# yhwu/rsicnv

Measured on AMD Instinct MI355X. Metric: bases/sec through RSI pipeline (bin+GC+NB+segment), higher is better.
Workload: dtype int32

## Files before the change

rsicnv_amd/csrc/kernels.h:

```cpp
#pragma once
#include <hip/hip_runtime.h>
#include <stdint.h>
#include <mutex>
#include "device_util.h"

namespace rsik {

inline void note_launch() {
  const hipError_t e = hipGetLastError();
  if (e != hipSuccess && tl_launch_error == hipSuccess) tl_launch_error = e;
}
inline void drain_stale_errors() { (void)hipGetLastError(); tl_launch_error = hipSuccess; }
inline hipError_t take_launch_error() { const hipError_t e = tl_launch_error; tl_launch_error = hipSuccess; return e; }
#define RSI_LAUNCH(...) do { hipLaunchKernelGGL(__VA_ARGS__); rsik::note_launch(); } while (0)

constexpr int kGcLevels = 202;
constexpr int kHistValues = 65536;
constexpr int kResClasses = 32;
constexpr int kTileBases = 4096;

void launch_fasta_classify(const uint8_t* fasta, int64_t n, uint64_t* gcbits, uint64_t* nbits, int64_t nwords,
                           const FillList& fill, hipStream_t stream);
void launch_fill(const FillList& fill, hipStream_t stream);
size_t fold_scratch_bytes();
// ... 185 lines not shown
#define RSI_ALLOW_FULL_LDS(kernel)                                                                                  \
  do {                                                                                                              \
    static std::once_flag once__[rsik::kMaxDevices];                                                                \
    int dev__ = 0;                                                                                                  \
    if (hipGetDevice(&dev__) != hipSuccess || dev__ < 0 || dev__ >= rsik::kMaxDevices) dev__ = 0;                   \
    std::call_once(once__[dev__], [dev__] {                                                                         \
      hipFuncAttributes a__;                                                                                        \
      int lds__ = 0;                                                                                                \
      if (hipFuncGetAttributes(&a__, reinterpret_cast<const void*>(kernel)) != hipSuccess) {                        \
        rsik::report_attribute_failure(#kernel, "hipFuncGetAttributes"); return;                                    \
      }                                                                                                             \
      if (hipDeviceGetAttribute(&lds__, hipDeviceAttributeMaxSharedMemoryPerBlock, dev__) != hipSuccess || lds__ <= 0) \
        lds__ = 160 * 1024;                                                                                         \
      if (hipFuncSetAttribute(reinterpret_cast<const void*>(kernel), hipFuncAttributeMaxDynamicSharedMemorySize,   \
                              lds__ - (int)a__.sharedSizeBytes) != hipSuccess)                                      \
        rsik::report_attribute_failure(#kernel, "hipFuncSetAttribute(MaxDynamicSharedMemorySize)");                 \
    });                                                                                                             \
  } while (0)

constexpr unsigned kCandHistBins = 16384;
struct EdgeJob {
  int32_t start, end, type, pad;
};
struct CandJob {
  int32_t start, end;
  int32_t kind;
  int32_t margin;
  int32_t capacity;
  int32_t top;
  int32_t nleft, nright;
  int32_t left_off, right_off;
  int32_t budget;
  int32_t cut;
  double right_cap;
  int64_t iscratch_off;
  int64_t lscratch_off;
};
struct CandOut {
  int32_t flags;
  int32_t nref, nbody, nwin, left_reach, right_reach, body_min, body_max;
  double body_q[3], body_s1, body_s2;
  double ref_q[3], ref_s1, ref_s2;
};
struct DepthRef { const void* p; int bytes; };
void launch_widen_u8(const uint8_t* src, int64_t n, int32_t* dst, hipStream_t stream);
void launch_patch_i32(int32_t* dst, const int32_t* pos, const int32_t* val, int64_t cnt, hipStream_t stream);
void launch_range_sums(DepthRef rdc, const void* ranges , int nranges, long long* sums, hipStream_t stream);
void launch_sharpen_edges(DepthRef rdc, int64_t ncompact, EdgeJob* jobs, int njobs, void* ws, int ws_jobs, hipStream_t stream);
size_t sharpen_workspace_bytes(int njobs);
size_t sharpen_workspace_zero_bytes(int njobs);
constexpr int kCandChunks = 16;
struct CandMid {
  int32_t lcnt, lreach, lused, rcnt_max, rreach, rused;
  uint32_t done, body_flags;
  long long totals[kCandChunks];
  float flo[kCandChunks], fhi[kCandChunks];
  double m1[kCandChunks], m2[kCandChunks];
  int32_t body_min, body_max;
  double body_q[3], body_s1, body_s2;
};
void launch_candidate_test_split(DepthRef rdc, int64_t ncompact, const CandJob* jobs, int njobs, const void* chains,
                                 int32_t* iscratch, long long* lscratch, double RDmedian, CandMid* mid, uint32_t* ghist,
                                 CandOut* outs, hipStream_t stream);
void launch_candidate_test(DepthRef rdc, int64_t ncompact, const CandJob* jobs, int njobs, const void* chains,
                           int32_t* iscratch, long long* lscratch, double RDmedian, CandOut* outs, hipStream_t stream);

struct TextParseStats { unsigned long long lines, stored, beyond; unsigned int unsorted, pad; };
int text_parse_workgroups(long long nbytes);
void launch_parse_depth_text(const void* text, long long nbytes, long long size, int32_t* depth, long long* wg_first,
                             long long* wg_max, TextParseStats* stats, hipStream_t stream);

struct NameBound { long long line; int32_t name, len; };
void launch_text_name_bounds(const void* text, long long nbytes, NameBound* bounds, unsigned int* count, unsigned int cap,
                             hipStream_t stream, bool bedgraph = false);
struct GenomeSeg { long long start, n; int32_t* depth; int32_t slot, pad; };
struct GenomeSlotStats { unsigned long long lines, stored, beyond; unsigned int unsorted, pad; long long last_pos;  };
constexpr int kMaxGenomeSegs = 512;
int genome_parse_workgroups(long long nbytes);
void launch_parse_genome_text(const void* text, long long begin, long long end, const GenomeSeg* segs, int nseg,
                              GenomeSlotStats* slots, long long* wg, hipStream_t stream);
constexpr int kMaxGenomeSamples = 64;
struct GenomeSampleCols { int32_t col[kMaxGenomeSamples], j[kMaxGenomeSamples]; int32_t n, pad; };
__host__ __device__ inline long long genome_sample_stride(long long n) { return (n + 4 + 3) & ~3ll; }
int genome_sample_parse_workgroups(long long nbytes);
void launch_parse_genome_samples(const void* text, long long begin, long long end, const GenomeSeg* segs, int nseg,
                                 const GenomeSampleCols& cols, GenomeSlotStats* slots, long long* wg, hipStream_t stream);
struct BedRun { int32_t* dst; uint32_t len; int32_t d; };
constexpr long long kBedPiece = 1ll << 20;
unsigned long long bedgraph_run_cap(long long text_bytes, long long sum_len);
void launch_parse_genome_bedgraph(const void* text, long long begin, long long end, const GenomeSeg* segs, int nseg, GenomeSlotStats* slots,
                                  long long* wg, BedRun* runs, unsigned long long* nruns, unsigned int run_cap, hipStream_t stream);

struct InflateBlock { long long coff, out; uint32_t clen, isize, crc, pad; };
void launch_inflate_bgzf(const void* comp, const InflateBlock* blocks, int nblocks, void* text, int* last_nl,
                         unsigned long long* status, hipStream_t stream);
void launch_gather_names(const void* text, const NameBound* bounds, unsigned k0, unsigned k1, char* out, hipStream_t stream);
// ... 9 lines not shown
```

rsicnv_amd/csrc/kernels_cand.hip:

```cpp
#include "kernels.h"

namespace rsik {

namespace {

constexpr int kThreads = 256;
constexpr int kTestThreads = 1024;
constexpr int kMaxWaves = kTestThreads / 64;
__device__ inline int lane_id() { return threadIdx.x & 63; }

template <class T, class Op>
__device__ inline T block_reduce(T v, Op op, T* s_tmp ) {
  for (int d = 32; d >= 1; d >>= 1) v = op(v, __shfl_xor(v, d));
  __syncthreads();
  if (lane_id() == 0) s_tmp[threadIdx.x >> 6] = v;
  __syncthreads();
  T r = s_tmp[0];
  for (int w = 1; w < (int)(blockDim.x >> 6); ++w) r = op(r, s_tmp[w]);
  __syncthreads();
  return r;
}
__device__ inline int block_exscan(int v, int* s_tmp , int* total) {
  const int incl = wave_incl_scan(v);
  __syncthreads();
  if (lane_id() == 63) s_tmp[threadIdx.x >> 6] = incl;
  __syncthreads();
  int base = 0, tot = 0;
  for (int w = 0; w < (int)(blockDim.x >> 6); ++w) { if (w < (int)(threadIdx.x >> 6)) base += s_tmp[w]; tot += s_tmp[w]; }
  __syncthreads();
  *total = tot;
  return base + incl - v;
}
template <class F>
// ... 143 lines not shown

constexpr int kWalkPer = 16;
constexpr int kWalkBlock = kWalkPer * kTestThreads;

struct WalkShared { int s_scan[kMaxWaves]; int cnt[2][kMaxWaves]; int trg[2][kMaxWaves]; int kept[2]; int lastt[2]; };

struct __attribute__((packed, aligned(1))) WalkBytes16 { uint32_t w[4]; };
struct __attribute__((packed, aligned(4))) WalkInts4 { int x, y, z, w; };
__device__ inline void walk_load16(const uint8_t* __restrict__ A, int64_t N, long long first, int dir, int* out) {
  const long long lo = dir > 0 ? first : first - 15;
  if (lo >= 0 && lo + 15 <= N - 1) {
    const WalkBytes16 b = *reinterpret_cast<const WalkBytes16*>(A + lo);
#pragma unroll
    for (int j = 0; j < 16; ++j) { const int k = dir > 0 ? j : 15 - j; out[j] = (int)((b.w[k >> 2] >> (8 * (k & 3))) & 0xffu); }
  } else {
#pragma unroll
    for (int j = 0; j < 16; ++j) { long long p = first + (long long)dir * j; p = p < 0 ? 0 : (p > N - 1 ? N - 1 : p); out[j] = (int)A[p]; }
  }
}
__device__ inline void walk_load16(const int32_t* __restrict__ A, int64_t N, long long first, int dir, int* out) {
  const long long lo = dir > 0 ? first : first - 15;
  if (lo >= 0 && lo + 15 <= N - 1) {
    int v[16];
#pragma unroll
    for (int q = 0; q < 4; ++q) { const WalkInts4 b = *reinterpret_cast<const WalkInts4*>(A + lo + 4 * q); v[4 * q] = b.x; v[4 * q + 1] = b.y; v[4 * q + 2] = b.z; v[4 * q + 3] = b.w; }
#pragma unroll
    for (int j = 0; j < 16; ++j) out[j] = v[dir > 0 ? j : 15 - j];
  } else {
#pragma unroll
    for (int j = 0; j < 16; ++j) { long long p = first + (long long)dir * j; p = p < 0 ? 0 : (p > N - 1 ? N - 1 : p); out[j] = A[p]; }
  }
}

template <typename TD>
__device__ inline int gather_side(const TD* __restrict__ A, int64_t N, int dir, int pos, int room ,
                                  int32_t* __restrict__ dst, int first_slot, const int2* __restrict__ chain, int nchain,
                                  int kind, double too_high, double too_low, WalkShared& W, int* reach, int* chain_used,
                                  int* __restrict__ stage ) {
  constexpr int kNone = 0x7fffffff;
  auto swz = [](int r) { return r ^ ((r >> 4) & 15); };
  int stored = 0, ci = 0, trip = 0;
  int last = pos;
  const int lane = lane_id(), wave = threadIdx.x >> 6, nwaves = blockDim.x >> 6;
  const double th = too_high > 2147483646.0 ? 2147483646.0 : (too_high < -2147483647.0 ? -2147483647.0 : floor(too_high));
  const double tl = too_low > 2147483646.0 ? 2147483646.0 : (too_low < -2147483647.0 ? -2147483647.0 : ceil(too_low));
  const int hi_lim = kind == 0 && too_high == too_high ? (too_high > 2147483646.0 ? 0x7fffffff : (int)th) : 0x7fffffff;
  const int lo_lim = kind == 1 && too_low == too_low ? (too_low < -2147483647.0 ? (int)0x80000000 : (int)tl) : (int)0x80000000;
  auto load16 = [&](int from, int* out) { walk_load16(A, N, (long long)from + (long long)dir * (1 + kWalkPer * (int)threadIdx.x), dir, out); };
  int vnext[kWalkPer];
  load16(pos, vnext);
  int2 cur = ci < nchain ? chain[ci] : make_int2(1, 0);
  while (room > 0 && (dir < 0 ? pos > 2 : (int64_t)pos < N - 2)) {
    const int par = trip & 1;
    ++trip;
    const int avail = dir < 0 ? pos - 2 : (int)(N - 2 - pos);
    const int cnt = avail < kWalkBlock ? avail : kWalkBlock;
    int v[kWalkPer]; unsigned accm = 0; int nacc = 0; int trig = kNone;
#pragma unroll
    for (int j = 0; j < kWalkPer; ++j) v[j] = vnext[j];
    load16(pos + dir * cnt, vnext);
    const int t0 = kWalkPer * (int)threadIdx.x;
#pragma unroll
    for (int j = 0; j < kWalkPer; ++j) {
      const int t = t0 + j;
      if (t < cnt) {
        const int p = pos + dir * (1 + t);
        const bool ext = v[j] > hi_lim || v[j] < lo_lim;
        const bool inside = p >= cur.x && p <= cur.y;
        if (!ext && inside && t < trig) trig = t;
        if (!ext && !inside) { accm |= 1u << j; ++nacc; }
      }
    }
    int incl = wave_incl_scan(nacc), wtrig = trig;
    for (int d = 32; d >= 1; d >>= 1) { const int o = __shfl_xor(wtrig, d); wtrig = o < wtrig ? o : wtrig; }
    if (lane == 63) W.cnt[par][wave] = incl;
    if (lane == 0) W.trg[par][wave] = wtrig;
    __syncthreads();
    int base = 0, all = 0, tstar = kNone;
    for (int w = 0; w < nwaves; ++w) { const int c = W.cnt[par][w]; if (w < wave) base += c; all += c; const int g = W.trg[par][w]; tstar = g < tstar ? g : tstar; }
    int rank = base + incl - nacc;
    int total = all;
    if (tstar != kNone) {
      if ((int)threadIdx.x == tstar / kWalkPer) {
        int k = rank;
#pragma unroll
        for (int j = 0; j < kWalkPer; ++j) if (((accm >> j) & 1u) && t0 + j < tstar) ++k;
        W.kept[par] = k;
      }
      __syncthreads();
// ... 294 lines not shown
  if (room < 0) room = 0;
  g.rcnt = M.rcnt_max < room ? M.rcnt_max : room;
  g.nref_raw = g.used0 + g.rcnt;
  g.nbody = J.end - J.start + 1;
  g.nref = g.nref_raw; g.nbody_eff = g.nbody; g.thin = false;
  if (g.nref_raw + g.nbody > J.budget) {
    const int total = g.nref_raw + g.nbody;
    g.nref = (int)((double)g.nref_raw / (double)total * (double)J.budget);
    g.nbody_eff = (int)((double)g.nbody / (double)total * (double)J.budget);
    g.thin = true;
  }
  g.width = g.nbody_eff;
  g.nwin = g.nref - g.width;
  return g;
}
struct CandBufs { int32_t *left, *ref, *thin, *right; long long* P; };
__device__ inline CandBufs cand_buffers(const CandJob& J, int32_t* iscratch, long long* lscratch) {
  CandBufs b;
  b.left = iscratch + J.iscratch_off;
  b.ref = b.left + (((J.top + 1 > 0 ? J.top + 1 : 0) + 3) & ~3);
  b.thin = b.ref + ((J.capacity + 3) & ~3);
  const int nthin = J.capacity < J.budget ? J.capacity : J.budget;
  b.right = b.thin + ((nthin + 3) & ~3);
  b.P = lscratch + J.lscratch_off;
  return b;
}
__device__ inline int cand_value(const CandJob& J, const CandGeom& g, const CandBufs& b, int i) {
  const int j = g.thin ? (int)((double)i / (double)g.nref * (double)g.nref_raw) : i;
  return j < g.used0 ? b.left[J.top + 1 - g.used0 + j] : b.right[j - g.used0];
}
__device__ inline int cand_chunk_len(int n) { return (((n + kCandChunks - 1) / kCandChunks) + 3) & ~3; }
constexpr int kCandP32MaxChunk = 16000000;

template <typename TD>
__global__ __launch_bounds__(kTestThreads) void k_cand_gather(const TD* __restrict__ A, int64_t N, const CandJob* __restrict__ jobs,
                                                          const int2* __restrict__ chains, int32_t* __restrict__ iscratch,
                                                          long long* __restrict__ lscratch, double RDmedian, CandMid* __restrict__ mid) {
  __shared__ WalkShared W;
  extern __shared__ int s_stage[];
  const CandJob J = jobs[blockIdx.y];
  const CandBufs b = cand_buffers(J, iscratch, lscratch);
  const double too_high = RDmedian * 3.0, too_low = RDmedian * 0.15;
  CandMid& M = mid[blockIdx.y];
  if (blockIdx.x == 0) {
    int lreach = J.start, lused = 0, lcnt = 0;
    if (J.top >= 0)
      lcnt = gather_side(A, N, -1, J.start - J.margin, J.top + 1, b.left, J.top, chains + J.left_off, J.nleft, J.kind, too_high, too_low, W, &lreach, &lused, s_stage);
    if (threadIdx.x == 0) { M.lcnt = lcnt; M.lreach = lreach; M.lused = lused; }
  } else {
    int room = J.capacity;
    const int lim = (int)ceil(J.right_cap);
    if (lim < room) room = lim;
    if ((J.cut & 4) && J.top >= 0) room -= J.top + 1;
    if (room < 0) room = 0;
    int rreach = J.end, rused = 0;
    const int rcnt = gather_side(A, N, +1, J.end + J.margin, room, b.right, 0, chains + J.right_off, J.nright, J.kind, too_high, too_low, W, &rreach, &rused, s_stage);
    if (threadIdx.x == 0) { M.rcnt_max = rcnt; M.rreach = rreach; M.rused = rused; }
  }
}

template <typename TD>
__global__ __launch_bounds__(kTestThreads) void k_cand_prefix(const TD* __restrict__ A, const CandJob* __restrict__ jobs,
                                                          int32_t* __restrict__ iscratch, long long* __restrict__ lscratch,
                                                          CandMid* __restrict__ mid) {
  extern __shared__ unsigned int s_hist[];
  __shared__ long long s_l[kMaxWaves];
  __shared__ int s_i2[kMaxWaves];
  __shared__ int s_scan[kMaxWaves];
  __shared__ int s_q[3];
  const CandJob J = jobs[blockIdx.y];
  CandMid& M = mid[blockIdx.y];
  const CandGeom g = cand_geometry(J, M);
  const CandBufs b = cand_buffers(J, iscratch, lscratch);
  if (g.nwin <= 0 || g.width <= 0) return;
  if (blockIdx.x < kCandChunks) {
    const int Lc = cand_chunk_len(g.nref);
    const int cb = blockIdx.x * Lc;
    int ce = cb + Lc; if (ce > g.nref) ce = g.nref;
    long long carry = 0;
    uint32_t* const P32 = reinterpret_cast<uint32_t*>(b.P);
    const bool p32 = sizeof(TD) == 1 && Lc <= kCandP32MaxChunk;
    if (blockIdx.x == 0 && threadIdx.x == 0) { if (p32) P32[0] = 0u; else b.P[0] = 0; }
    constexpr int kPer = 16;
    for (int t0 = cb; t0 < ce; t0 += kPer * kTestThreads) {
      const int e = t0 + kPer * (int)threadIdx.x;
      int v[kPer];
      if (!g.thin && e + kPer <= ce && (e + kPer <= g.used0 || e >= g.used0)) {
        const int32_t* src = e < g.used0 ? b.left + (J.top + 1 - g.used0 + e) : b.right + (e - g.used0);
#pragma unroll
        for (int q = 0; q < 4; ++q) { const WalkInts4 w4 = *reinterpret_cast<const WalkInts4*>(src + 4 * q); v[4 * q] = w4.x; v[4 * q + 1] = w4.y; v[4 * q + 2] = w4.z; v[4 * q + 3] = w4.w; }
      } else {
// ... 125 lines not shown
  const int Wc = cand_chunk_len(g.nwin);
  const int wb = blockIdx.x * Wc;
  int we = wb + Wc; if (we > g.nwin) we = g.nwin;
  float* Wm = reinterpret_cast<float*>(b.ref);
  const double dw = (double)g.width;
  float flo = 3.0e38f, fhi = -3.0e38f; double m1 = 0, m2 = 0;
  for (int q = wb + (int)threadIdx.x; q < we; q += kTestThreads) {
    const float w = (float)((double)(P_at(q + g.width) - P_at(q)) / dw);
    Wm[q] = w;
    flo = w < flo ? w : flo; fhi = w > fhi ? w : fhi; m1 += (double)w; m2 += (double)w * (double)w;
  }
  flo = block_reduce(flo, [](float a, float b2) { return a < b2 ? a : b2; }, s_f);
  fhi = block_reduce(fhi, [](float a, float b2) { return a > b2 ? a : b2; }, s_f);
  m1 = block_reduce(m1, [](double a, double b2) { return a + b2; }, s_d);
  m2 = block_reduce(m2, [](double a, double b2) { return a + b2; }, s_d);
  if (threadIdx.x == 0) { M.flo[blockIdx.x] = flo; M.fhi[blockIdx.x] = fhi; M.m1[blockIdx.x] = m1; M.m2[blockIdx.x] = m2; }
}

__global__ __launch_bounds__(kTestThreads) void k_cand_hist(const CandJob* __restrict__ jobs, int32_t* __restrict__ iscratch,
                                                        long long* __restrict__ lscratch, CandMid* __restrict__ mid,
                                                        uint32_t* __restrict__ ghist_all, CandOut* __restrict__ outs) {
  extern __shared__ unsigned int s_hist[];
  __shared__ int s_scan[kMaxWaves];
  __shared__ int s_q[3];
  __shared__ int s_last;
  const CandJob J = jobs[blockIdx.y];
  CandMid& M = mid[blockIdx.y];
  const CandGeom g = cand_geometry(J, M);
  const CandBufs b = cand_buffers(J, iscratch, lscratch);
  uint32_t* ghist = ghist_all + (size_t)blockIdx.y * kCandHistBins;
  CandOut O;
  O.flags = M.body_flags;
  if (((J.cut & 1) && M.lused >= J.nleft) || ((J.cut & 2) && M.rused >= J.nright)) O.flags |= 8;
  if ((J.cut & 4) && J.top >= 0 && M.lcnt < J.top + 1) O.flags |= 16;
  O.nref = g.nref; O.nbody = g.nbody_eff; O.nwin = g.nwin; O.left_reach = M.lreach; O.right_reach = M.rreach;
  if (g.nwin <= 0 || g.width <= 0) {
    O.flags = (O.flags & 24) | 1;
    O.body_min = O.body_max = 0; O.body_s1 = O.body_s2 = O.ref_s1 = O.ref_s2 = 0;
    for (int k = 0; k < 3; ++k) { O.body_q[k] = 0; O.ref_q[k] = 0; }
    if (blockIdx.x == 0 && threadIdx.x == 0) outs[blockIdx.y] = O;
    return;
  }
  O.body_min = M.body_min; O.body_max = M.body_max; O.body_s1 = M.body_s1; O.body_s2 = M.body_s2;
  O.body_q[0] = M.body_q[0]; O.body_q[1] = M.body_q[1]; O.body_q[2] = M.body_q[2];
  float flo = 3.0e38f, fhi = -3.0e38f; double m1 = 0, m2 = 0;
  for (int c = 0; c < kCandChunks; ++c) {
    flo = M.flo[c] < flo ? M.flo[c] : flo; fhi = M.fhi[c] > fhi ? M.fhi[c] : fhi; m1 += M.m1[c]; m2 += M.m2[c];
  }
  const double lo = flo, hi = fhi;
  O.ref_s1 = m1; O.ref_s2 = m2;
  O.ref_q[0] = lo; O.ref_q[1] = m1 / (double)g.nwin; O.ref_q[2] = hi;
  const bool spread = (hi - lo) >= 0.01;
  const size_t nbk = spread ? (size_t)((hi - lo) / 0.01 + 2) : 0;
  if (!spread || nbk > kCandHistBins) {
    if (spread) O.flags |= 4;
    if (blockIdx.x == 0 && threadIdx.x == 0) outs[blockIdx.y] = O;
    return;
  }
  const float* Wm = reinterpret_cast<const float*>(b.ref);
  for (unsigned e = threadIdx.x; e < nbk; e += kTestThreads) s_hist[e] = 0;
  __syncthreads();
  const int Wc = cand_chunk_len(g.nwin);
  const int wb = blockIdx.x * Wc;
  int we = wb + Wc; if (we > g.nwin) we = g.nwin;
  for (int i0 = wb + 8 * (int)threadIdx.x; i0 < we; i0 += 8 * kTestThreads) {
    unsigned pend_b = 0xffffffffu, pend_c = 0;
#pragma unroll
// ... 25 lines not shown
}

template <typename TD>
__global__ __launch_bounds__(kThreads) void k_range_sums(const TD* __restrict__ A, const int2* __restrict__ ranges,
                                                         long long* __restrict__ sums) {
  __shared__ long long s_l[kThreads / 64 + 1];
  const int2 r = ranges[blockIdx.x];
  long long acc = 0;
  for (int p = r.x + (int)threadIdx.x; p <= r.y; p += kThreads) acc += A[p];
  acc = block_reduce(acc, [](long long a, long long b) { return a + b; }, s_l);
  if (threadIdx.x == 0) sums[blockIdx.x] = acc;
}

}

#define RSI_DEPTH_DISPATCH(D, CALL32, CALL8) do { if ((D).bytes == 1) { const uint8_t* rdc = static_cast<const uint8_t*>((D).p); CALL8; } \
                                                 else { const int32_t* rdc = static_cast<const int32_t*>((D).p); CALL32; } } while (0)

void launch_range_sums(DepthRef d, const void* ranges, int nranges, long long* sums, hipStream_t stream) {
  if (nranges <= 0) return;
  RSI_DEPTH_DISPATCH(d,
    RSI_LAUNCH(k_range_sums<int32_t>, dim3(nranges), dim3(kThreads), 0, stream, rdc, static_cast<const int2*>(ranges), sums),
    RSI_LAUNCH(k_range_sums<uint8_t>, dim3(nranges), dim3(kThreads), 0, stream, rdc, static_cast<const int2*>(ranges), sums));
}

void launch_sharpen_edges(DepthRef d, int64_t ncompact, EdgeJob* jobs, int njobs, void* ws, int ws_jobs, hipStream_t stream) {
  if (njobs <= 0) return;
  RSI_DEPTH_DISPATCH(d,
    RSI_LAUNCH(k_sharpen_edges<int32_t>, dim3(2 * kEdgeChunks, njobs), dim3(kThreads), 0, stream, rdc, ncompact, jobs, ws_jobs, ws),
    RSI_LAUNCH(k_sharpen_edges<uint8_t>, dim3(2 * kEdgeChunks, njobs), dim3(kThreads), 0, stream, rdc, ncompact, jobs, ws_jobs, ws));
}
void launch_candidate_test_split(DepthRef d, int64_t ncompact, const CandJob* jobs, int njobs, const void* chains,
                                 int32_t* iscratch, long long* lscratch, double RDmedian, CandMid* mid, uint32_t* ghist,
                                 CandOut* outs, hipStream_t stream) {
  if (njobs <= 0) return;
  const size_t lds = (size_t)kCandHistBins * 4;
  static_assert(kCandHistBins * 4 >= (unsigned)kWalkBlock * 4, "the walks stage a trip in the histogram's LDS");
  RSI_ALLOW_FULL_LDS(k_cand_gather<int32_t>);
  RSI_ALLOW_FULL_LDS(k_cand_gather<uint8_t>);
  RSI_ALLOW_FULL_LDS(k_cand_prefix<int32_t>);
  RSI_ALLOW_FULL_LDS(k_cand_prefix<uint8_t>);
  RSI_ALLOW_FULL_LDS(k_cand_hist);
  const int2* ch = static_cast<const int2*>(chains);
  RSI_DEPTH_DISPATCH(d,
    RSI_LAUNCH(k_cand_gather<int32_t>, dim3(2, njobs), dim3(kTestThreads), lds, stream, rdc, ncompact, jobs, ch, iscratch, lscratch, RDmedian, mid),
    RSI_LAUNCH(k_cand_gather<uint8_t>, dim3(2, njobs), dim3(kTestThreads), lds, stream, rdc, ncompact, jobs, ch, iscratch, lscratch, RDmedian, mid));
  RSI_DEPTH_DISPATCH(d,
    RSI_LAUNCH(k_cand_prefix<int32_t>, dim3(kCandChunks + 1, njobs), dim3(kTestThreads), lds, stream, rdc, jobs, iscratch, lscratch, mid),
    RSI_LAUNCH(k_cand_prefix<uint8_t>, dim3(kCandChunks + 1, njobs), dim3(kTestThreads), lds, stream, rdc, jobs, iscratch, lscratch, mid));
  RSI_LAUNCH(k_cand_means, dim3(kCandChunks, njobs), dim3(kTestThreads), 0, stream, jobs, iscratch, lscratch, mid, d.bytes == 1 ? 1 : 0);
  RSI_LAUNCH(k_cand_hist, dim3(kCandChunks, njobs), dim3(kTestThreads), lds, stream, jobs, iscratch, lscratch, mid, ghist, outs);
}
size_t sharpen_workspace_bytes(int njobs) { return sharpen_zero_bytes(njobs) + (size_t)njobs * 2 * kEdgeChunks * (8 + 8 + 4); }
size_t sharpen_workspace_zero_bytes(int njobs) { return sharpen_zero_bytes(njobs); }
void launch_candidate_test(DepthRef d, int64_t ncompact, const CandJob* jobs, int njobs, const void* chains,
                           int32_t* iscratch, long long* lscratch, double RDmedian, CandOut* outs, hipStream_t stream) {
  if (njobs <= 0) return;
  const size_t lds = (size_t)kCandHistBins * 4;
  RSI_ALLOW_FULL_LDS(k_candidate_test<int32_t>);
  RSI_ALLOW_FULL_LDS(k_candidate_test<uint8_t>);
  RSI_DEPTH_DISPATCH(d,
    RSI_LAUNCH(k_candidate_test<int32_t>, dim3(njobs), dim3(kTestThreads), lds, stream, rdc, ncompact, jobs, static_cast<const int2*>(chains), iscratch, lscratch, RDmedian, outs),
    RSI_LAUNCH(k_candidate_test<uint8_t>, dim3(njobs), dim3(kTestThreads), lds, stream, rdc, ncompact, jobs, static_cast<const int2*>(chains), iscratch, lscratch, RDmedian, outs));
}
#undef RSI_DEPTH_DISPATCH

__global__ __launch_bounds__(256) void k_widen_u8(const uint8_t* __restrict__ src, int64_t n, int32_t* __restrict__ dst) {
  const int64_t i0 = ((int64_t)blockIdx.x * 256 + threadIdx.x) * 16;
  if (i0 + 16 <= n) {
    const uint4 b = *reinterpret_cast<const uint4*>(src + i0);
    const uint32_t w[4] = {b.x, b.y, b.z, b.w};
#pragma unroll
    for (int q = 0; q < 4; ++q)
      *reinterpret_cast<int4*>(dst + i0 + 4 * q) = make_int4((int)(w[q] & 0xffu), (int)((w[q] >> 8) & 0xffu), (int)((w[q] >> 16) & 0xffu), (int)(w[q] >> 24));
  } else {
    for (int64_t i = i0; i < n; ++i) dst[i] = (int)src[i];
  }
}
void launch_widen_u8(const uint8_t* src, int64_t n, int32_t* dst, hipStream_t stream) {
  if (n <= 0) return;
  const int64_t blocks = (n + 256 * 16 - 1) / (256 * 16);
  RSI_LAUNCH(k_widen_u8, dim3((unsigned int)blocks), dim3(256), 0, stream, src, n, dst);
}

__global__ __launch_bounds__(256) void k_patch_i32(int32_t* __restrict__ dst, const int32_t* __restrict__ pos, const int32_t* __restrict__ val, int64_t cnt) {
  for (int64_t k = (int64_t)blockIdx.x * 256 + threadIdx.x; k < cnt; k += (int64_t)gridDim.x * 256) dst[pos[k]] = val[k];
}
void launch_patch_i32(int32_t* dst, const int32_t* pos, const int32_t* val, int64_t cnt, hipStream_t stream) {
  if (cnt <= 0) return;
  const int64_t blocks = std::min<int64_t>((cnt + 255) / 256, 1024);
  RSI_LAUNCH(k_patch_i32, dim3((unsigned int)blocks), dim3(256), 0, stream, dst, pos, val, cnt);
// ... 4 lines not shown
```

rsicnv_amd/csrc/pipeline.hip:

```cpp
#include <new>
#include "pipeline_internal.h"

using namespace rsik;
using namespace rsip;
using rsih::Candidate;
using rsih::Region;

namespace {

struct ScanPassOut { uint32_t escapes, inexact, ldel, ldup; };

struct ScanOut {
  double tmedian1 = 0, tsigma1 = 0, tlamda1 = 0, tmedian2 = 0, tsigma2 = 0, tlamda2 = 0;
  int Lmax = 0;
  rsih::IntSpan status2;
  std::vector<int> run_status;
  std::vector<rsih::IntSpan::Range> run_ranges;
  std::vector<Candidate> segs;
  uint32_t escapes = 0, inexact = 0;
  uint32_t tiles_listed = 0;
  std::vector<uint32_t> level_log[4];
  uint32_t stop_levels[4] = {0, 0, 0, 0};
  std::vector<std::string> fs_lines;
};
// ... 201 lines not shown
        if (!ok(ctx->sharpen_ws.ensure(sharpen_workspace_bytes(cap)))) return false;
        if (!ok(hipMemsetAsync(ctx->sharpen_ws.p, 0, sharpen_workspace_zero_bytes(cap), ctx->stream))) return false;
        ctx->sharpen_ws_jobs = cap;
      }
      if (!slot && !ok(ctx->cand_jobs.ensure((size_t)nj * sizeof(EdgeJob)))) return false;
    }
    GateShared gs(ctx);
    Phase ph(ctx, "cand.sharpen");
    EdgeJob* d_jobs = slot ? slot : ctx->cand_jobs.as<EdgeJob>();
    if (!slot && !ok(copy_h2d(ctx, ctx->cand_jobs.p, jobs, (size_t)nj * sizeof(EdgeJob)))) return false;
    for (int pass = 0; pass < 2; ++pass) {
      Timer t(ctx, "sharpen_edges");
      launch_sharpen_edges(d_rdc, N, d_jobs, nj, ctx->sharpen_ws.p, ctx->sharpen_ws_jobs, ctx->stream);
    }
    if (!slot && !ok(copy_d2h(ctx, jobs, ctx->cand_jobs.p, (size_t)nj * sizeof(EdgeJob)))) return false;
    if (!wait()) return false;
    gs.release();
    for (int i = 0; i < nj; ++i) { L[(size_t)i].start = jobs[i].start; L[(size_t)i].end = jobs[i].end; }
    return true;
  }

  bool test(const std::vector<rsih::TestPlan>& plans, std::vector<rsih::TestStats>& stats, std::vector<int>& left_reach,
            std::vector<char>& okv) override {
    const size_t n = plans.size();
    stats.assign(n, rsih::TestStats{});
    left_reach.assign(n, 0);
    okv.assign(n, 0);
    const bool split = env_int("RSI_HOT_CAND_SPLIT", 1) != 0;
    size_t first = 0;
    while (first < n) {
      std::vector<CandJob> jobs;
      std::vector<int32_t> chains;
      size_t iwords = 0, lwords = 0, last = first;
      for (; last < n; ++last) {
        const rsih::TestPlan& T = plans[last];
        if (T.capacity <= 0 || T.end < T.start || T.start < 0 || T.end >= N) break;
        auto up4 = [](size_t x) { return (x + 3) & ~(size_t)3; };
        const size_t iw = up4((size_t)std::max(T.top + 1, 0)) + up4((size_t)T.capacity) + up4((size_t)std::min(T.capacity, T.budget)) +
                          (split ? up4((size_t)T.capacity) : 0);
        const size_t lw = up4((size_t)T.capacity + 1);
        if (!jobs.empty() && (iwords + iw) * 4 + (lwords + lw) * 8 > kCandScratchBytes) break;
        CandJob J{};
        J.start = T.start; J.end = T.end; J.kind = T.kind; J.margin = T.margin; J.capacity = T.capacity; J.top = T.top;
        J.nleft = (int)T.left_chain.size(); J.nright = (int)T.right_chain.size();
        J.left_off = (int)(chains.size() / 2);
        for (const auto& iv : T.left_chain) { chains.push_back(iv.first); chains.push_back(iv.second); }
        J.right_off = (int)(chains.size() / 2);
        for (const auto& iv : T.right_chain) { chains.push_back(iv.first); chains.push_back(iv.second); }
        J.budget = T.budget; J.cut = T.cut; J.right_cap = T.right_cap;
        J.iscratch_off = (int64_t)iwords; J.lscratch_off = (int64_t)lwords;
        iwords += iw; lwords += lw;
        jobs.push_back(J);
      }
      if (jobs.empty()) { ++first; continue; }
      chains.push_back(0); chains.push_back(0);
      std::vector<CandOut> outs(jobs.size());
      {
        Phase ph(ctx, "cand.ensure");
        if (!ok(ctx->cand_jobs.ensure(jobs.size() * sizeof(CandJob))) || !ok(ctx->cand_chains.ensure(chains.size() * 4)) ||
            !ok(ctx->cand_outs.ensure(outs.size() * sizeof(CandOut))) || !ok(ctx->cand_i32.ensure(iwords * 4)) ||
            !ok(ctx->cand_i64.ensure(lwords * 8)))
          return false;
        if (split) {
          const size_t m0 = ctx->cand_mid.cap, h0 = ctx->cand_hist.cap;
          if (!ok(ctx->cand_mid.ensure(jobs.size() * sizeof(CandMid))) || !ok(ctx->cand_hist.ensure(jobs.size() * (size_t)kCandHistBins * 4))) return false;
          if (ctx->cand_mid.cap != m0 && !ok(hipMemsetAsync(ctx->cand_mid.p, 0, ctx->cand_mid.cap, ctx->stream))) return false;
          if (ctx->cand_hist.cap != h0 && !ok(hipMemsetAsync(ctx->cand_hist.p, 0, ctx->cand_hist.cap, ctx->stream))) return false;
        }
      }
      GateShared gs(ctx);
      Phase ph(ctx, "cand.test");
      const size_t jb = (jobs.size() * sizeof(CandJob) + 63) & ~size_t(63), cb = (chains.size() * 4 + 63) & ~size_t(63);
      const size_t ob = outs.size() * sizeof(CandOut);
      unsigned char* slot = jb + cb + ob <= kMailboxMaxCopy ? static_cast<unsigned char*>(mb_alloc(ctx, jb + cb + ob)) : nullptr;
      const CandJob* d_jobs = ctx->cand_jobs.as<CandJob>();
      const void* d_chains = ctx->cand_chains.p;
      CandOut* d_outs = ctx->cand_outs.as<CandOut>();
      if (slot) {
        memcpy(slot, jobs.data(), jobs.size() * sizeof(CandJob));
        memcpy(slot + jb, chains.data(), chains.size() * 4);
        d_jobs = reinterpret_cast<const CandJob*>(slot); d_chains = slot + jb; d_outs = reinterpret_cast<CandOut*>(slot + jb + cb);
      } else {
        if (!ok(copy_h2d(ctx, ctx->cand_jobs.p, jobs.data(), jobs.size() * sizeof(CandJob)))) return false;
        if (!ok(copy_h2d(ctx, ctx->cand_chains.p, chains.data(), chains.size() * 4))) return false;
      }
      {
        Timer t(ctx, split ? "candidate_test" : "candidate_test_one_wg");
        if (split)
          launch_candidate_test_split(d_rdc, N, d_jobs, (int)jobs.size(), d_chains, ctx->cand_i32.as<int32_t>(),
                                      ctx->cand_i64.as<long long>(), median, ctx->cand_mid.as<CandMid>(), ctx->cand_hist.as<uint32_t>(),
                                      d_outs, ctx->stream);
        else
          launch_candidate_test(d_rdc, N, d_jobs, (int)jobs.size(), d_chains, ctx->cand_i32.as<int32_t>(),
                                ctx->cand_i64.as<long long>(), median, d_outs, ctx->stream);
      }
      if (!slot && !ok(copy_d2h(ctx, outs.data(), ctx->cand_outs.p, outs.size() * sizeof(CandOut)))) return false;
      if (!wait()) return false;
      if (slot) memcpy(outs.data(), d_outs, ob);
      gs.release();
      ph.stop();
      static const bool cand_dbg = env_int("RSI_HOT_CAND_DBG", 0) != 0;
      for (size_t k = 0; k < jobs.size(); ++k) {
        const CandOut& O = outs[k];
        if (cand_dbg)
          fprintf(stderr, "[cand] [%d,%d] kind %d margin %d cap %d top %d chains %d/%d cut %d -> flags %d nref %d nbody %d nwin %d reach %d/%d ref q %.6f %.6f %.6f s1 %.6f s2 %.6f\n",
                  jobs[k].start, jobs[k].end, jobs[k].kind, jobs[k].margin, jobs[k].capacity, jobs[k].top, jobs[k].nleft, jobs[k].nright, jobs[k].cut,
                  O.flags, O.nref, O.nbody, O.nwin, O.left_reach, O.right_reach, O.ref_q[0], O.ref_q[1], O.ref_q[2], O.ref_s1, O.ref_s2);
        if (O.flags != 0) continue;
        rsih::TestStats& S = stats[first + k];
        const double nb = (double)O.nbody, nw = (double)O.nwin;
        S.cnv_lqt = O.body_q[0]; S.cnv_med = O.body_q[1]; S.cnv_uqt = O.body_q[2];
        { const double mu = O.body_s1 / nb; S.cnv_var = O.body_s2 / nb - mu * mu; }
        S.ref_lqt = O.ref_q[0]; S.ref_med = O.ref_q[1]; S.ref_uqt = O.ref_q[2];
        { const double mu = O.ref_s1 / nw; S.ref_var = O.ref_s2 / nw - mu * mu; }
        left_reach[first + k] = O.left_reach;
        okv[first + k] = 1;
      }
      first += jobs.size();
    }
    return true;
  }

  bool range_sums(const std::vector<std::pair<int, int>>& ranges, std::vector<int64_t>& sums) override {
    sums.assign(ranges.size(), 0);
    if (ranges.empty()) return true;
    std::vector<int32_t> flat;
    for (const auto& r : ranges) {
      if (r.first < 0 || r.second >= N || r.second < r.first) return false;
      flat.push_back(r.first); flat.push_back(r.second);
    }
    static_assert(sizeof(long long) == sizeof(int64_t), "int64");
    const size_t fb = (flat.size() * 4 + 63) & ~size_t(63);
    unsigned char* slot = static_cast<unsigned char*>(mb_alloc(ctx, fb + ranges.size() * 8));
    GateShared gs(ctx);
    if (slot) {
      memcpy(slot, flat.data(), flat.size() * 4);
      long long* d_sums = reinterpret_cast<long long*>(slot + fb);
      { Timer t(ctx, "range_sums"); launch_range_sums(d_rdc, slot, (int)ranges.size(), d_sums, ctx->stream); }
      if (!wait()) return false;
      memcpy(sums.data(), d_sums, ranges.size() * 8);
// ... 1422 lines not shown
```

Measured before the change: 214.9 billion.

## Parallelize candidate gather walk across tiles with count/scan/scatter kernels

Replaces the two-block-per-job sequential gather walk with a tiled count kernel that counts kept samples per 4096-base tile across many blocks. A last-arriving block scans the tile counts to find where room is filled, resolves chain triggers, and falls back to the old sequential walk when chains overflow or overlap. A separate scatter kernel then writes each tile's kept values at its scanned offset. The host precomputes per-job tile counts to size the grid. The aim is to expose far more parallelism for long walks, at the cost of an extra launch, atomics and more complex fallback logic; one overflow flag is also dropped.

Measured after the change: 208.8 billion (median of 2 runs). -2.8%, worse.

```diff
diff --git a/rsicnv_amd/csrc/kernels.h b/rsicnv_amd/csrc/kernels.h
--- a/rsicnv_amd/csrc/kernels.h
+++ b/rsicnv_amd/csrc/kernels.h
@@ -241,6 +241,7 @@
   int32_t left_off, right_off;
   int32_t budget;
   int32_t cut;
+  int32_t tiles[2];
   double right_cap;
   int64_t iscratch_off;
   int64_t lscratch_off;
@@ -259,9 +260,16 @@
 size_t sharpen_workspace_bytes(int njobs);
 size_t sharpen_workspace_zero_bytes(int njobs);
 constexpr int kCandChunks = 16;
+constexpr int kCandChainMax = 48;
+constexpr int kCandGatherTile = 4096;
 struct CandMid {
   int32_t lcnt, lreach, lused, rcnt_max, rreach, rused;
   uint32_t done, body_flags;
+  uint32_t gdone;
+  int32_t gmode[2];
+  int32_t gstop[2], groom[2];
+  uint32_t walked;
+  uint32_t trig[2][kCandChainMax];
   long long totals[kCandChunks];
   float flo[kCandChunks], fhi[kCandChunks];
   double m1[kCandChunks], m2[kCandChunks];
@@ -270,7 +278,8 @@
 };
 void launch_candidate_test_split(DepthRef rdc, int64_t ncompact, const CandJob* jobs, int njobs, const void* chains,
                                  int32_t* iscratch, long long* lscratch, double RDmedian, CandMid* mid, uint32_t* ghist,
-                                 CandOut* outs, hipStream_t stream);
+                                 CandOut* outs, int max_tiles, hipStream_t stream);
+int cand_gather_tiles(const CandJob& J, const int2* chains, int64_t ncompact, int side);
 void launch_candidate_test(DepthRef rdc, int64_t ncompact, const CandJob* jobs, int njobs, const void* chains,
                            int32_t* iscratch, long long* lscratch, double RDmedian, CandOut* outs, hipStream_t stream);
 
diff --git a/rsicnv_amd/csrc/kernels_cand.hip b/rsicnv_amd/csrc/kernels_cand.hip
--- a/rsicnv_amd/csrc/kernels_cand.hip
+++ b/rsicnv_amd/csrc/kernels_cand.hip
@@ -1,4 +1,7 @@
 #include "kernels.h"
+
+#include <algorithm>
+#include <cmath>
 
 namespace rsik {
 
@@ -208,6 +211,13 @@
   }
 }
 
+__device__ inline void extreme_limits(int kind, double too_high, double too_low, int* hi_lim, int* lo_lim) {
+  const double th = too_high > 2147483646.0 ? 2147483646.0 : (too_high < -2147483647.0 ? -2147483647.0 : floor(too_high));
+  const double tl = too_low > 2147483646.0 ? 2147483646.0 : (too_low < -2147483647.0 ? -2147483647.0 : ceil(too_low));
+  *hi_lim = kind == 0 && too_high == too_high ? (too_high > 2147483646.0 ? 0x7fffffff : (int)th) : 0x7fffffff;
+  *lo_lim = kind == 1 && too_low == too_low ? (too_low < -2147483647.0 ? (int)0x80000000 : (int)tl) : (int)0x80000000;
+}
+
 template <typename TD>
 __device__ inline int gather_side(const TD* __restrict__ A, int64_t N, int dir, int pos, int room ,
                                   int32_t* __restrict__ dst, int first_slot, const int2* __restrict__ chain, int nchain,
@@ -218,10 +228,8 @@
   int stored = 0, ci = 0, trip = 0;
   int last = pos;
   const int lane = lane_id(), wave = threadIdx.x >> 6, nwaves = blockDim.x >> 6;
-  const double th = too_high > 2147483646.0 ? 2147483646.0 : (too_high < -2147483647.0 ? -2147483647.0 : floor(too_high));
-  const double tl = too_low > 2147483646.0 ? 2147483646.0 : (too_low < -2147483647.0 ? -2147483647.0 : ceil(too_low));
-  const int hi_lim = kind == 0 && too_high == too_high ? (too_high > 2147483646.0 ? 0x7fffffff : (int)th) : 0x7fffffff;
-  const int lo_lim = kind == 1 && too_low == too_low ? (too_low < -2147483647.0 ? (int)0x80000000 : (int)tl) : (int)0x80000000;
+  int hi_lim, lo_lim;
+  extreme_limits(kind, too_high, too_low, &hi_lim, &lo_lim);
   auto load16 = [&](int from, int* out) { walk_load16(A, N, (long long)from + (long long)dir * (1 + kWalkPer * (int)threadIdx.x), dir, out); };
   int vnext[kWalkPer];
   load16(pos, vnext);
@@ -230,7 +238,8 @@
     const int par = trip & 1;
     ++trip;
     const int avail = dir < 0 ? pos - 2 : (int)(N - 2 - pos);
-    const int cnt = avail < kWalkBlock ? avail : kWalkBlock;
+    const int trip_len = kWalkPer * (int)blockDim.x;
+    const int cnt = avail < trip_len ? avail : trip_len;
     int v[kWalkPer]; unsigned accm = 0; int nacc = 0; int trig = kNone;
 #pragma unroll
     for (int j = 0; j < kWalkPer; ++j) v[j] = vnext[j];
@@ -591,31 +600,246 @@
 __device__ inline int cand_chunk_len(int n) { return (((n + kCandChunks - 1) / kCandChunks) + 3) & ~3; }
 constexpr int kCandP32MaxChunk = 16000000;
 
+constexpr int kGatherThreads = kCandGatherTile / kWalkPer;
+static_assert(kCandChainMax <= kGatherThreads, "one thread per chain entry");
+struct GatherTileShared {
+  int4 ent[kCandChainMax];
+  int trig[kCandChainMax];
+  int nent;
+  int scan[kMaxWaves];
+  int misc[4];
+};
+struct GatherWalk { int dir, pos0, avail, nchain; const int2* chain; };
+__device__ inline GatherWalk gather_walk(const CandJob& J, int side, int64_t N, const int2* chains) {
+  GatherWalk g;
+  g.dir = side == 0 ? -1 : 1;
+  g.pos0 = side == 0 ? J.start - J.margin : J.end + J.margin;
+  g.avail = side == 0 ? g.pos0 - 2 : (int)(N - 2 - g.pos0);
+  g.chain = chains + (side == 0 ? J.left_off : J.right_off);
+  g.nchain = side == 0 ? J.nleft : J.nright;
+  return g;
+}
+__device__ inline int2 entry_walk(const GatherWalk& g, int2 e) {
+  return g.dir < 0 ? make_int2(g.pos0 - 1 - e.y, g.pos0 - 1 - e.x) : make_int2(e.x - g.pos0 - 1, e.y - g.pos0 - 1);
+}
+__device__ inline int walk_pos(const GatherWalk& g, int t) { return g.pos0 + g.dir * (1 + t); }
+__device__ inline void tile_entries(const GatherWalk& g, int T0, int T1, GatherTileShared& s) {
+  if (threadIdx.x == 0) s.nent = 0;
+  __syncthreads();
+  const int nch = g.nchain < kCandChainMax ? g.nchain : kCandChainMax;
+  if ((int)threadIdx.x < nch) {
+    const int2 w = entry_walk(g, g.chain[threadIdx.x]);
+    if (w.x < T1 && w.y + 1 >= T0) {
+      const int k = atomicAdd(&s.nent, 1);
+      s.ent[k] = make_int4(w.x, w.y, (int)threadIdx.x, 0);
+      s.trig[k] = 0x7fffffff;
+    }
+  }
+  __syncthreads();
+}
+template <typename TD, bool kTrig>
+__device__ inline unsigned tile_taken(const TD* __restrict__ A, int64_t N, const GatherWalk& g, int t0, int T1, int hi_lim, int lo_lim,
+                                      GatherTileShared& s, int* v) {
+  walk_load16(A, N, (long long)walk_pos(g, t0), g.dir, v);
+  unsigned ext = 0;
+#pragma unroll
+  for (int j = 0; j < kWalkPer; ++j) if (t0 + j >= T1 || v[j] > hi_lim || v[j] < lo_lim) ext |= 1u << j;
+  unsigned m = ~ext & 0xffffu;
+  for (int k = 0; k < s.nent; ++k) {
+    const int4 e = s.ent[k];
+    const int a = e.x - t0, bb = e.y + 1 - t0;
+    if (bb < 0 || a >= kWalkPer) continue;
+    const int lo = a < 0 ? 0 : a, hi = bb > kWalkPer - 1 ? kWalkPer - 1 : bb;
+    const unsigned span = ((2u << hi) - 1u) & ~((1u << lo) - 1u);
+    if (kTrig) {
+      const unsigned core = span & ~(bb <= kWalkPer - 1 ? (1u << bb) : 0u);
+      const unsigned ne = ~ext & core & 0xffffu;
+      if (ne) atomicMin(&s.trig[k], t0 + __builtin_ctz(ne));
+    }
+    m &= ~span;
+  }
+  return m;
+}
+
 template <typename TD>
-__global__ __launch_bounds__(kTestThreads) void k_cand_gather(const TD* __restrict__ A, int64_t N, const CandJob* __restrict__ jobs,
-                                                          const int2* __restrict__ chains, int32_t* __restrict__ iscratch,
-                                                          long long* __restrict__ lscratch, double RDmedian, CandMid* __restrict__ mid) {
+__global__ __launch_bounds__(kGatherThreads) void k_cand_count(const TD* __restrict__ A, int64_t N, const CandJob* __restrict__ jobs,
+                                                           const int2* __restrict__ chains, int32_t* __restrict__ iscratch,
+                                                           long long* __restrict__ lscratch, double RDmedian, CandMid* __restrict__ mid) {
+  __shared__ GatherTileShared s;
   __shared__ WalkShared W;
   extern __shared__ int s_stage[];
-  const CandJob J = jobs[blockIdx.y];
+  const int side = blockIdx.y, tile = blockIdx.x;
+  const CandJob J = jobs[blockIdx.z];
+  if (tile >= J.tiles[side]) return;
+  CandMid& M = mid[blockIdx.z];
   const CandBufs b = cand_buffers(J, iscratch, lscratch);
+  int32_t* const counts = reinterpret_cast<int32_t*>(b.P);
   const double too_high = RDmedian * 3.0, too_low = RDmedian * 0.15;
-  CandMid& M = mid[blockIdx.y];
-  if (blockIdx.x == 0) {
-    int lreach = J.start, lused = 0, lcnt = 0;
-    if (J.top >= 0)
-      lcnt = gather_side(A, N, -1, J.start - J.margin, J.top + 1, b.left, J.top, chains + J.left_off, J.nleft, J.kind, too_high, too_low, W, &lreach, &lused, s_stage);
-    if (threadIdx.x == 0) { M.lcnt = lcnt; M.lreach = lreach; M.lused = lused; }
-  } else {
-    int room = J.capacity;
-    const int lim = (int)ceil(J.right_cap);
-    if (lim < room) room = lim;
-    if ((J.cut & 4) && J.top >= 0) room -= J.top + 1;
-    if (room < 0) room = 0;
-    int rreach = J.end, rused = 0;
-    const int rcnt = gather_side(A, N, +1, J.end + J.margin, room, b.right, 0, chains + J.right_off, J.nright, J.kind, too_high, too_low, W, &rreach, &rused, s_stage);
-    if (threadIdx.x == 0) { M.rcnt_max = rcnt; M.rreach = rreach; M.rused = rused; }
-  }
+  int hi_lim, lo_lim;
+  extreme_limits(J.kind, too_high, too_low, &hi_lim, &lo_lim);
+  {
+    const GatherWalk g = gather_walk(J, side, N, chains);
+    const int T0 = tile * kCandGatherTile;
+    const int T1 = g.avail - T0 < kCandGatherTile ? g.avail : T0 + kCandGatherTile;
+    int c = 0;
+    if (T1 > T0 && !(side == 0 && J.top < 0)) {
+      tile_entries(g, T0, T1, s);
+      int v[kWalkPer];
+      c = __builtin_popcount(tile_taken<TD, true>(A, N, g, T0 + kWalkPer * (int)threadIdx.x, T1, hi_lim, lo_lim, s, v));
+      int tot;
+      block_exscan(c, s.scan, &tot);
+      c = tot;
+      if ((int)threadIdx.x < s.nent && s.trig[threadIdx.x] != 0x7fffffff)
+        atomicMax(&M.trig[side][s.ent[threadIdx.x].z], 0x7fffffffu - (unsigned)s.trig[threadIdx.x]);
+    }
+    if (threadIdx.x == 0) st_cg(reinterpret_cast<unsigned int*>(&counts[side * J.tiles[0] + tile]), (unsigned int)c);
+  }
+  drain();
+  __syncthreads();
+  if (threadIdx.x == 0) s.misc[0] = atomicAdd(&M.gdone, 1u) == (unsigned)(J.tiles[0] + J.tiles[1] - 1);
+  __syncthreads();
+  if (!s.misc[0]) return;
+
+  int lcnt = 0;
+  unsigned walked = 0;
+  for (int sd = 0; sd < 2; ++sd) {
+    const GatherWalk g = gather_walk(J, sd, N, chains);
+    int room;
+    if (sd == 0) room = J.top >= 0 ? J.top + 1 : 0;
+    else {
+      const int used0 = J.top >= 0 ? (lcnt < J.top + 1 ? lcnt : J.top + 1) : 0;
+      room = J.capacity - used0;
+      const int lim = (int)ceil(J.right_cap);
+      if (lim - used0 < room) room = lim - used0;
+      if (room < 0) room = 0;
+    }
+    const int nt = J.tiles[sd];
+    int32_t* const cnt_sd = counts + sd * J.tiles[0];
+    int cnt = 0, reach = g.pos0, used = 0, mode = 0, stop_tile = -1;
+    const int nch = g.nchain < kCandChainMax ? g.nchain : kCandChainMax;
+    if (sd == 0 && J.top < 0) reach = J.start;
+    else if (room > 0 && g.avail > 0) {
+      if (threadIdx.x == 0) { s.misc[1] = -1; s.misc[2] = 0; }
+      int carry = 0;
+      for (int t0 = 0; t0 < nt; t0 += kGatherThreads) {
+        const int t = t0 + (int)threadIdx.x;
+        const int c = t < nt ? (int)ld_cg(reinterpret_cast<const unsigned int*>(&cnt_sd[t])) : 0;
+        int tot;
+        const int ex = carry + block_exscan(c, s.scan, &tot);
+        if (t < nt) {
+          cnt_sd[t] = ex;
+          if (c > 0 && ex < room && ex + c >= room) { s.misc[1] = t; s.misc[2] = ex; }
+        }
+        carry += tot;
+      }
+      __syncthreads();
+      const int T = s.misc[1], offT = s.misc[2];
+      __syncthreads();
+      const bool filled = T >= 0;
+      bool walk = g.nchain > kCandChainMax || (!filled && (long long)nt * kCandGatherTile < g.avail);
+      int stop_t = g.avail - 1;
+      if (filled) {
+        const int T0 = T * kCandGatherTile;
+        const int T1 = g.avail - T0 < kCandGatherTile ? g.avail : T0 + kCandGatherTile;
+        tile_entries(g, T0, T1, s);
+        int v[kWalkPer];
+        const int t0 = T0 + kWalkPer * (int)threadIdx.x;
+        const unsigned m = tile_taken<TD, false>(A, N, g, t0, T1, hi_lim, lo_lim, s, v);
+        int tot;
+        const int base = block_exscan(__builtin_popcount(m), s.scan, &tot);
+        const int r = room - 1 - offT;
+        if (r >= base && r < base + __builtin_popcount(m)) {
+          unsigned mm = m;
+          for (int k = base; k < r; ++k) mm &= mm - 1;
+          s.misc[3] = t0 + __builtin_ctz(mm);
+        }
+        __syncthreads();
+        stop_t = s.misc[3];
+        __syncthreads();
+      }
+      if (threadIdx.x == 0) { s.misc[1] = nch; s.misc[2] = 0; }
+      __syncthreads();
+      unsigned tv = 0;
+      int2 w = make_int2(0, -2);
+      if ((int)threadIdx.x < nch) {
+        tv = __hip_atomic_load(&M.trig[sd][threadIdx.x], __ATOMIC_RELAXED, __HIP_MEMORY_SCOPE_AGENT);
+        s.trig[threadIdx.x] = tv ? 0x7fffffff - (int)tv : -1;
+        if (!tv) atomicMin(&s.misc[1], (int)threadIdx.x);
+        w = entry_walk(g, g.chain[threadIdx.x]);
+      }
+      __syncthreads();
+      const int jstar = s.misc[1];
+      if ((int)threadIdx.x < nch && w.x <= stop_t && w.y + 1 >= 0) {
+        bool bad = (int)threadIdx.x >= jstar;
+        if (threadIdx.x > 0) { const int2 pw = entry_walk(g, g.chain[threadIdx.x - 1]); bad = bad || w.x <= pw.y + 1; }
+        if (bad) s.misc[2] = 1;
+      }
+      __syncthreads();
+      walk = walk || s.misc[2] != 0;
+      if (!walk) {
+        cnt = filled ? room : carry;
+        for (int j = 0; j < jstar && s.trig[j] <= stop_t; ++j) used = j + 1;
+        if (filled) reach = walk_pos(g, stop_t);
+        else {
+          reach = walk_pos(g, g.avail - 1);
+          if (used > 0) {
+            const int2 lw = entry_walk(g, g.chain[used - 1]);
+            if (lw.y + 1 >= g.avail - 1) reach = walk_pos(g, s.trig[used - 1]);
+          }
+        }
+        mode = 1;
+        stop_tile = filled ? T : nt - 1;
+      } else {
+        walked |= 1u << sd;
+        cnt = gather_side(A, N, g.dir, g.pos0, room, sd == 0 ? b.left : b.right, sd == 0 ? J.top : 0, g.chain, g.nchain, J.kind,
+                          too_high, too_low, W, &reach, &used, s_stage);
+      }
+    }
+    if ((int)threadIdx.x < kCandChainMax) M.trig[sd][threadIdx.x] = 0;
+    if (threadIdx.x == 0) {
+      M.gmode[sd] = mode; M.gstop[sd] = stop_tile; M.groom[sd] = room;
+      if (sd == 0) { M.lcnt = cnt; M.lreach = reach; M.lused = used; }
+      else { M.rcnt_max = cnt; M.rreach = reach; M.rused = used; }
+    }
+    if (sd == 0) lcnt = cnt;
+    __syncthreads();
+  }
+  if (threadIdx.x == 0) { M.walked = walked; M.gdone = 0; }
+}
+
+template <typename TD>
+__global__ __launch_bounds__(kGatherThreads) void k_cand_scatter(const TD* __restrict__ A, int64_t N, const CandJob* __restrict__ jobs,
+                                                             const int2* __restrict__ chains, int32_t* __restrict__ iscratch,
+                                                             long long* __restrict__ lscratch, double RDmedian, const CandMid* __restrict__ mid) {
+  __shared__ GatherTileShared s;
+  __shared__ int s_vals[kCandGatherTile];
+  const int side = blockIdx.y, tile = blockIdx.x;
+  const CandJob J = jobs[blockIdx.z];
+  if (tile >= J.tiles[side]) return;
+  const CandMid& M = mid[blockIdx.z];
+  if (M.gmode[side] != 1 || tile > M.gstop[side]) return;
+  const CandBufs b = cand_buffers(J, iscratch, lscratch);
+  const int off = reinterpret_cast<const int32_t*>(b.P)[side * J.tiles[0] + tile];
+  const int room = M.groom[side];
+  if (off >= room) return;
+  const GatherWalk g = gather_walk(J, side, N, chains);
+  const int T0 = tile * kCandGatherTile;
+  const int T1 = g.avail - T0 < kCandGatherTile ? g.avail : T0 + kCandGatherTile;
+  if (T1 <= T0) return;
+  int hi_lim, lo_lim;
+  extreme_limits(J.kind, RDmedian * 3.0, RDmedian * 0.15, &hi_lim, &lo_lim);
+  tile_entries(g, T0, T1, s);
+  int v[kWalkPer];
+  const unsigned m = tile_taken<TD, false>(A, N, g, T0 + kWalkPer * (int)threadIdx.x, T1, hi_lim, lo_lim, s, v);
+  int tot;
+  int rank = block_exscan(__builtin_popcount(m), s.scan, &tot);
+  auto swz = [](int r) { return r ^ ((r >> 4) & 15); };
+#pragma unroll
+  for (int j = 0; j < kWalkPer; ++j) if ((m >> j) & 1u) s_vals[swz(rank++)] = v[j];
+  __syncthreads();
+  const int n = tot < room - off ? tot : room - off;
+  if (side == 0) { int32_t* dst = b.left + J.top - off; for (int e = threadIdx.x; e < n; e += kGatherThreads) dst[-e] = s_vals[swz(e)]; }
+  else { int32_t* dst = b.right + off; for (int e = threadIdx.x; e < n; e += kGatherThreads) dst[e] = s_vals[swz(e)]; }
 }
 
 template <typename TD>
@@ -807,7 +1031,6 @@
   CandOut O;
   O.flags = M.body_flags;
   if (((J.cut & 1) && M.lused >= J.nleft) || ((J.cut & 2) && M.rused >= J.nright)) O.flags |= 8;
-  if ((J.cut & 4) && J.top >= 0 && M.lcnt < J.top + 1) O.flags |= 16;
   O.nref = g.nref; O.nbody = g.nbody_eff; O.nwin = g.nwin; O.left_reach = M.lreach; O.right_reach = M.rreach;
   if (g.nwin <= 0 || g.width <= 0) {
     O.flags = (O.flags & 24) | 1;
@@ -899,24 +1122,48 @@
 }
 void launch_candidate_test_split(DepthRef d, int64_t ncompact, const CandJob* jobs, int njobs, const void* chains,
                                  int32_t* iscratch, long long* lscratch, double RDmedian, CandMid* mid, uint32_t* ghist,
-                                 CandOut* outs, hipStream_t stream) {
+                                 CandOut* outs, int max_tiles, hipStream_t stream) {
   if (njobs <= 0) return;
   const size_t lds = (size_t)kCandHistBins * 4;
-  static_assert(kCandHistBins * 4 >= (unsigned)kWalkBlock * 4, "the walks stage a trip in the histogram's LDS");
-  RSI_ALLOW_FULL_LDS(k_cand_gather<int32_t>);
-  RSI_ALLOW_FULL_LDS(k_cand_gather<uint8_t>);
+  const size_t walk_lds = (size_t)kCandGatherTile * 4;
   RSI_ALLOW_FULL_LDS(k_cand_prefix<int32_t>);
   RSI_ALLOW_FULL_LDS(k_cand_prefix<uint8_t>);
   RSI_ALLOW_FULL_LDS(k_cand_hist);
   const int2* ch = static_cast<const int2*>(chains);
+  const dim3 gg(max_tiles > 1 ? max_tiles : 1, 2, njobs);
   RSI_DEPTH_DISPATCH(d,
-    RSI_LAUNCH(k_cand_gather<int32_t>, dim3(2, njobs), dim3(kTestThreads), lds, stream, rdc, ncompact, jobs, ch, iscratch, lscratch, RDmedian, mid),
-    RSI_LAUNCH(k_cand_gather<uint8_t>, dim3(2, njobs), dim3(kTestThreads), lds, stream, rdc, ncompact, jobs, ch, iscratch, lscratch, RDmedian, mid));
+    RSI_LAUNCH(k_cand_count<int32_t>, gg, dim3(kGatherThreads), walk_lds, stream, rdc, ncompact, jobs, ch, iscratch, lscratch, RDmedian, mid),
+    RSI_LAUNCH(k_cand_count<uint8_t>, gg, dim3(kGatherThreads), walk_lds, stream, rdc, ncompact, jobs, ch, iscratch, lscratch, RDmedian, mid));
+  RSI_DEPTH_DISPATCH(d,
+    RSI_LAUNCH(k_cand_scatter<int32_t>, gg, dim3(kGatherThreads), 0, stream, rdc, ncompact, jobs, ch, iscratch, lscratch, RDmedian, mid),
+    RSI_LAUNCH(k_cand_scatter<uint8_t>, gg, dim3(kGatherThreads), 0, stream, rdc, ncompact, jobs, ch, iscratch, lscratch, RDmedian, mid));
   RSI_DEPTH_DISPATCH(d,
     RSI_LAUNCH(k_cand_prefix<int32_t>, dim3(kCandChunks + 1, njobs), dim3(kTestThreads), lds, stream, rdc, jobs, iscratch, lscratch, mid),
     RSI_LAUNCH(k_cand_prefix<uint8_t>, dim3(kCandChunks + 1, njobs), dim3(kTestThreads), lds, stream, rdc, jobs, iscratch, lscratch, mid));
   RSI_LAUNCH(k_cand_means, dim3(kCandChunks, njobs), dim3(kTestThreads), 0, stream, jobs, iscratch, lscratch, mid, d.bytes == 1 ? 1 : 0);
   RSI_LAUNCH(k_cand_hist, dim3(kCandChunks, njobs), dim3(kTestThreads), lds, stream, jobs, iscratch, lscratch, mid, ghist, outs);
+}
+int cand_gather_tiles(const CandJob& J, const int2* chains, int64_t ncompact, int side) {
+  if (side == 0 && J.top < 0) return 1;
+  const int dir = side == 0 ? -1 : 1;
+  const long long pos0 = side == 0 ? (long long)J.start - J.margin : (long long)J.end + J.margin;
+  const long long avail = side == 0 ? pos0 - 2 : ncompact - 2 - pos0;
+  long long room = std::min<long long>(J.capacity, (long long)std::ceil(J.right_cap));
+  if (side == 0) room = J.top + 1;
+  else if ((J.cut & 4) && J.top >= 0) room -= J.top + 1;
+  if (avail <= 0 || room <= 0) return 1;
+  long long span = room + room / 8 + kCandGatherTile;
+  const int2* ch = chains + (side == 0 ? J.left_off : J.right_off);
+  const int nch = side == 0 ? J.nleft : J.nright;
+  for (int j = 0; j < nch; ++j) {
+    const long long ca = dir < 0 ? pos0 - 1 - ch[j].y : ch[j].x - pos0 - 1, cb = dir < 0 ? pos0 - 1 - ch[j].x : ch[j].y - pos0 - 1;
+    if (cb < 0) continue;
+    if (ca >= span) break;
+    span += cb - std::max(ca, 0ll) + 2;
+  }
+  span = std::min(span, avail);
+  const long long tiles = (span + kCandGatherTile - 1) / kCandGatherTile;
+  return (int)std::max(1ll, std::min({tiles, (long long)J.capacity + 1, 4096ll}));
 }
 size_t sharpen_workspace_bytes(int njobs) { return sharpen_zero_bytes(njobs) + (size_t)njobs * 2 * kEdgeChunks * (8 + 8 + 4); }
 size_t sharpen_workspace_zero_bytes(int njobs) { return sharpen_zero_bytes(njobs); }
@@ -924,6 +1171,7 @@
                            int32_t* iscratch, long long* lscratch, double RDmedian, CandOut* outs, hipStream_t stream) {
   if (njobs <= 0) return;
   const size_t lds = (size_t)kCandHistBins * 4;
+  static_assert(kCandHistBins * 4 >= (unsigned)kWalkBlock * 4, "the walks stage a trip in the histogram's LDS");
   RSI_ALLOW_FULL_LDS(k_candidate_test<int32_t>);
   RSI_ALLOW_FULL_LDS(k_candidate_test<uint8_t>);
   RSI_DEPTH_DISPATCH(d,
diff --git a/rsicnv_amd/csrc/pipeline.hip b/rsicnv_amd/csrc/pipeline.hip
--- a/rsicnv_amd/csrc/pipeline.hip
+++ b/rsicnv_amd/csrc/pipeline.hip
@@ -257,6 +257,7 @@
       std::vector<CandJob> jobs;
       std::vector<int32_t> chains;
       size_t iwords = 0, lwords = 0, last = first;
+      int max_tiles = 1;
       for (; last < n; ++last) {
         const rsih::TestPlan& T = plans[last];
         if (T.capacity <= 0 || T.end < T.start || T.start < 0 || T.end >= N) break;
@@ -274,6 +275,11 @@
         for (const auto& iv : T.right_chain) { chains.push_back(iv.first); chains.push_back(iv.second); }
         J.budget = T.budget; J.cut = T.cut; J.right_cap = T.right_cap;
         J.iscratch_off = (int64_t)iwords; J.lscratch_off = (int64_t)lwords;
+        if (split)
+          for (int sd = 0; sd < 2; ++sd) {
+            J.tiles[sd] = cand_gather_tiles(J, reinterpret_cast<const int2*>(chains.data()), N, sd);
+            max_tiles = std::max(max_tiles, J.tiles[sd]);
+          }
         iwords += iw; lwords += lw;
         jobs.push_back(J);
       }
@@ -314,7 +320,7 @@
         if (split)
           launch_candidate_test_split(d_rdc, N, d_jobs, (int)jobs.size(), d_chains, ctx->cand_i32.as<int32_t>(),
                                       ctx->cand_i64.as<long long>(), median, ctx->cand_mid.as<CandMid>(), ctx->cand_hist.as<uint32_t>(),
-                                      d_outs, ctx->stream);
+                                      d_outs, max_tiles, ctx->stream);
         else
           launch_candidate_test(d_rdc, N, d_jobs, (int)jobs.size(), d_chains, ctx->cand_i32.as<int32_t>(),
                                 ctx->cand_i64.as<long long>(), median, d_outs, ctx->stream);
@@ -325,12 +331,18 @@
       gs.release();
       ph.stop();
       static const bool cand_dbg = env_int("RSI_HOT_CAND_DBG", 0) != 0;
+      std::vector<CandMid> mids;
+      if (cand_dbg && split) {
+        mids.resize(jobs.size());
+        if (!ok(hipMemcpy(mids.data(), ctx->cand_mid.p, mids.size() * sizeof(CandMid), hipMemcpyDeviceToHost))) return false;
+      }
       for (size_t k = 0; k < jobs.size(); ++k) {
         const CandOut& O = outs[k];
         if (cand_dbg)
-          fprintf(stderr, "[cand] [%d,%d] kind %d margin %d cap %d top %d chains %d/%d cut %d -> flags %d nref %d nbody %d nwin %d reach %d/%d ref q %.6f %.6f %.6f s1 %.6f s2 %.6f\n",
+          fprintf(stderr, "[cand] [%d,%d] kind %d margin %d cap %d top %d chains %d/%d cut %d -> flags %d nref %d nbody %d nwin %d reach %d/%d ref q %.6f %.6f %.6f s1 %.6f s2 %.6f walked %d\n",
                   jobs[k].start, jobs[k].end, jobs[k].kind, jobs[k].margin, jobs[k].capacity, jobs[k].top, jobs[k].nleft, jobs[k].nright, jobs[k].cut,
-                  O.flags, O.nref, O.nbody, O.nwin, O.left_reach, O.right_reach, O.ref_q[0], O.ref_q[1], O.ref_q[2], O.ref_s1, O.ref_s2);
+                  O.flags, O.nref, O.nbody, O.nwin, O.left_reach, O.right_reach, O.ref_q[0], O.ref_q[1], O.ref_q[2], O.ref_s1, O.ref_s2,
+                  split ? (int)mids[k].walked : -1);
         if (O.flags != 0) continue;
         rsih::TestStats& S = stats[first + k];
         const double nb = (double)O.nbody, nw = (double)O.nwin;
```
